# ocrickard/piper-swift

Measured on AMD Instinct MI355X. Metric: audio-sec/wall-sec (RTF^-1) with ms/utterance, Piper VITS en_GB-medium geometry, scale-bench factor, higher is better.
Workload: dtype f32; 1 GPU; medium factor=8: 112 ids, 336 frames, 86016 samples (3.901 s audio) per utterance, 1 utterance per step per GPU; factor=8, phoneme_count=112, frames=336, samples=86016, parallelism=utterance-replicas x1 (one-shot RCCL weight broadcast)

## Files before the change

### piper-swift_amd/csrc/conv_win.h

```cpp
#pragma once
#include "common.h"

namespace ph {

struct ConvWinArgs {
  const float* x = nullptr;
  const float* x2 = nullptr;
  const float* x3 = nullptr;
  const float* w4 = nullptr;
  const float* bias = nullptr;
  const float* res = nullptr;
  const float* mrf_a = nullptr;
  const float* mrf_b = nullptr;
  float* y = nullptr;
  float pro_alpha = 1.0f;
  float out_alpha = 1.0f;
  int N = 1, Cin = 0, Cout = 0, K = 1, dil = 1, padL = 0;
  int Lin = 0;
  int Lout = 0;
  int y_len = 0;
  int ct_stride = 0, ct_pad = 0;
  const int* len_ptr = nullptr;
  int len_mul = 1;
};

size_t packed_conv_win_floats(int Cout, int Cin, int K);
size_t packed_convt_win_floats(int Cin, int Cout, int K, int stride);
int pack_conv_weights_win(hipStream_t s, const float* w, int Cout, int Cin, int K, float* packed);
int pack_convt_weights_win(hipStream_t s, const float* w, int Cin, int Cout, int K, int stride, int pad, float* packed);

bool conv_win_eligible(int Cout, int Cin, int K, int dil, int padL, int Lin, int Lout);
bool convt_win_eligible(int Cin, int Cout, int K, int stride, int pad, int Lin);

int launch_conv_win(piper_hip_ctx* ctx, hipStream_t s, const ConvWinArgs& a);
constexpr int kWinMulti = 3;
int launch_conv_win_multi(piper_hip_ctx* ctx, hipStream_t s, const ConvWinArgs* convs, int count);

size_t packed_conv_pipe_floats(int Cout, int Cin, int K);
size_t packed_convt_pipe_floats(int Cin, int Cout, int K, int stride);
int pack_conv_weights_pipe(hipStream_t s, const float* w, int Cout, int Cin, int K, float* packed);
int pack_convt_weights_pipe(hipStream_t s, const float* w, int Cin, int Cout, int K, int stride, int pad, float* packed);
bool conv_pipe_eligible(int Cout, int Cin, int K, int dil, int padL, int Lin, int Lout);
bool convt_pipe_eligible(int Cin, int Cout, int K, int stride, int pad, int Lin);
int launch_conv_pipe_multi(piper_hip_ctx* ctx, hipStream_t s, const ConvWinArgs* convs, int count);

struct RbPairArgs {
  const float* x = nullptr;
  float* y = nullptr;
  const float *wa4 = nullptr, *ba = nullptr, *wb4 = nullptr, *bb = nullptr;
  int Ka = 1, dila = 1, Kb = 1, dilb = 1;
  int res_a = 1, res_b_x = 0;
  float alpha = 0.1f;
  int N = 1, C = 0, L = 0;
  const int* len_ptr = nullptr;
  int len_mul = 1;
};
bool rb_pair_eligible(int C, int Ka, int dila, int Kb, int dilb, int L);
int launch_rb_pair_multi(piper_hip_ctx* ctx, hipStream_t s, const RbPairArgs* pairs, int count);

}
```

### piper-swift_amd/csrc/conv_win.hip

```cpp
#include <algorithm>
#include <cstdlib>
#include <type_traits>

#include "conv_win.h"

namespace ph {
namespace {

typedef float f32x16 __attribute__((ext_vector_type(16)));

constexpr int kBT = 256;
constexpr int kRA = 8;
constexpr int kStepPad = 16;
constexpr int kTailFloats = 4096;

__device__ __forceinline__ float lrelu1(float v, float alpha) { return v >= 0.0f ? v : v * alpha; }

inline int padded_steps_win(int Cin, int taps) { return (taps * (Cin / 2) + kStepPad - 1) / kStepPad * kStepPad; }

__global__ __launch_bounds__(kBT) void pack_conv_win_kernel(const float* __restrict__ w, int Cout, int Cin, int K, int S, int Sp,
                                                           float* __restrict__ out, int64_t total) {
  const int C2 = Cin >> 1;
  for (int64_t i = (int64_t)blockIdx.x * kBT + threadIdx.x; i < total; i += (int64_t)gridDim.x * kBT) {
    const int e = (int)(i & 3), l = (int)((i >> 2) & 63);
    const int64_t g = i >> 8;
    const int s4 = (int)(g % (Sp >> 2)), mt = (int)(g / (Sp >> 2));
    const int step = 4 * s4 + e;
    float v = 0.0f;
    const int row = mt * 32 + (l & 31);
    if (step < S && row < Cout) {
      const int tap = step / C2, c2 = step - tap * C2;
      v = w[((int64_t)row * Cin + 2 * c2 + (l >> 5)) * K + tap];
    }
    out[i] = v;
  }
}

__global__ __launch_bounds__(kBT) void pack_convt_win_kernel(const float* __restrict__ w, int Cin, int Cout, int K, int stride, int pad,
                                                            int S, int Sp, float* __restrict__ out, int64_t total) {
  const int C2 = Cin >> 1;
  for (int64_t i = (int64_t)blockIdx.x * kBT + threadIdx.x; i < total; i += (int64_t)gridDim.x * kBT) {
    const int e = (int)(i & 3), l = (int)((i >> 2) & 63);
    const int64_t g = i >> 8;
    const int s4 = (int)(g % (Sp >> 2)), mt = (int)(g / (Sp >> 2));
    const int step = 4 * s4 + e;
    float v = 0.0f;
    const int R = mt * 32 + (l & 31);
    const int rho = R / Cout, co = R - rho * Cout;
    if (step < S && rho < stride) {
      const int j = step / C2, c2 = step - j * C2;
      v = w[((int64_t)(2 * c2 + (l >> 5)) * Cout + co) * K + (rho + pad) % stride + stride * j];
    }
    out[i] = v;
  }
}

#ifdef PH_WIN_TRACE
__device__ unsigned long long* ph_win_trace_buf;
#define PH_WSTAMP(k) do { const int bl_ = blockIdx.x + gridDim.x * (blockIdx.y + gridDim.y * blockIdx.z); if ((threadIdx.x & 63) == 0 && ph_win_trace_buf && bl_ < 1024) ph_win_trace_buf[((size_t)bl_ * 4 + (threadIdx.x >> 6)) * 8 + (k)] = __builtin_amdgcn_s_memtime(); } while (0)
#else
#define PH_WSTAMP(k) do { } while (0)
#endif

struct ConvWinMulti {
  ConvWinArgs c[kWinMulti];
};

template <int WM, int WN, int KS>
__global__ __launch_bounds__(64 * WM * WN * KS) void conv_win_kernel(const ConvWinMulti multi, int batch, int xcd_rows) {
  constexpr int NW = WM * WN * KS, BT = 64 * NW;
  extern __shared__ __attribute__((aligned(16))) float win[];
  const ConvWinArgs& p = multi.c[blockIdx.z / batch];
  int bx = blockIdx.x, by = blockIdx.y;
  if (xcd_rows) {
    const int lin = blockIdx.x + gridDim.x * blockIdx.y;
    const int q = lin >> 3;
    const int yh = __builtin_amdgcn_readfirstlane(q / (int)gridDim.x);
    bx = q - yh * (int)gridDim.x;
    by = (lin & 7) + 8 * yh;
  }
  static_assert(NW == 4 || NW == 8, "4 or 8 waves per block");
  constexpr int NBC = WN * 32;
  PH_WSTAMP(0);
  const int lane = threadIdx.x & 63;
  const int wave = __builtin_amdgcn_readfirstlane(threadIdx.x >> 6);
  const int ks = wave / (WM * WN), wt = wave % (WM * WN);
  const int wm = wt % WM, wn = wt / WM;
  const int r = lane & 31, h = lane >> 5;
  const bool ct = p.ct_stride > 0;
  const int taps = ct ? p.K / p.ct_stride : p.K;
  const int C2 = p.Cin >> 1;
  const int n = blockIdx.z % batch;
  const int nb0 = bx * NBC;
  if (p.len_ptr && nb0 >= min(p.len_ptr[n] * p.len_mul, p.Lin)) return;
  const int mt = by * WM + wm;
  const int off_min = ct ? -(taps - 1) : -p.padL;
  const int off_max = ct ? (p.ct_stride - 1 + p.ct_pad) / p.ct_stride : (p.K - 1) * p.dil - p.padL;
  const int W = NBC + off_max - off_min;
  const int g0 = nb0 + off_min;
  const int ga = g0 & ~3;
  const int shift = g0 - ga;
  const int Wp = (W + 3 + 3) & ~3;
  const int S = taps * C2;
  const int Sp = (S + kStepPad - 1) / kStepPad * kStepPad;
  const int Sw = Sp / KS;
  const int s_begin = ks * Sw;

  const char* wa = (const char*)p.w4 + ((int64_t)mt * Sp + s_begin) * 256;
  const unsigned lane16 = (unsigned)lane * 16u;
  float4 a[kRA];
  auto load_a = [&](int slot, int ahead) { a[slot] = *(const float4*)(wa + ahead * 1024 + lane16); };
#pragma unroll
  for (int d = 0; d < kRA - 1; d++) load_a(d, d);

  auto stage = [&](auto avg_tag) {
    constexpr bool AVG = decltype(avg_tag)::value;
    constexpr int kStage = (AVG ? 5 : 16) * 4 / NW + (AVG && NW > 4 ? 1 : 0);
    const int64_t xoff = (int64_t)n * p.Cin * p.Lin;
    const float* xb = p.x + xoff;
    const float* xb2 = AVG ? p.x2 + xoff : nullptr;
    const float* xb3 = AVG ? p.x3 + xoff : nullptr;
    const int W4 = Wp >> 2;
    const int total4 = p.Cin * W4;
    const int dump = p.Cin * Wp;
    const int Lv = p.len_ptr ? min(p.len_ptr[n] * p.len_mul, p.Lin) : p.Lin;
    const unsigned inv = 0xFFFFFFFFu / (unsigned)W4 + 1u;
    for (int base = threadIdx.x; base < total4; base += BT * kStage) {
      float4 t[kStage], t2[AVG ? kStage : 1], t3[AVG ? kStage : 1];
// ... 6 lines not shown
        const int row = (int)__umulhi((unsigned)ic, inv);
        const int i4 = ic - row * W4;
        const int pos = ga + 4 * i4;
        nvalid[q] = pos < 0 ? 0 : Lv - pos;
        const int64_t off = (int64_t)row * p.Lin + ((pos >= 0 && pos < p.Lin) ? pos : 0);
        t[q] = *(const float4*)(xb + off);
        if constexpr (AVG) { t2[q] = *(const float4*)(xb2 + off); t3[q] = *(const float4*)(xb3 + off); }
        dst[q] = i < total4 ? row * Wp + 4 * i4 : dump;
      }
#pragma unroll
      for (int q = 0; q < kStage; q++) {
        float4 v = t[q];
        if constexpr (AVG) {
          v.x = ((v.x + t2[q].x) + t3[q].x) / 3.0f; v.y = ((v.y + t2[q].y) + t3[q].y) / 3.0f;
          v.z = ((v.z + t2[q].z) + t3[q].z) / 3.0f; v.w = ((v.w + t2[q].w) + t3[q].w) / 3.0f;
        }
        v.x = lrelu1(v.x, p.pro_alpha); v.y = lrelu1(v.y, p.pro_alpha); v.z = lrelu1(v.z, p.pro_alpha); v.w = lrelu1(v.w, p.pro_alpha);
        v.x = nvalid[q] > 0 ? v.x : 0.0f; v.y = nvalid[q] > 1 ? v.y : 0.0f; v.z = nvalid[q] > 2 ? v.z : 0.0f; v.w = nvalid[q] > 3 ? v.w : 0.0f;
        *(float4*)(win + dst[q]) = v;
      }
    }
  };
  PH_WSTAMP(1);
  if (p.x2) stage(std::true_type{});
  else stage(std::false_type{});
  PH_WSTAMP(2);
  __syncthreads();
  PH_WSTAMP(3);

  f32x16 acc;
#pragma unroll
  for (int q = 0; q < 16; q++) acc[q] = 0.0f;

  const int rho = ct ? (mt * 32) / p.Cout : 0;
  const int off0 = ct ? (rho + p.ct_pad) / p.ct_stride : -p.padL;
  const int dstep = ct ? -1 : p.dil;
  const int lbase = h * Wp + shift + wn * 32 + r - off_min + off0;
  const int tap0 = s_begin / C2, c20 = s_begin - tap0 * C2;
  int sidx = 2 * c20 * Wp + min(tap0, taps - 1) * dstep;
  int c_n = c20, left = S - 1 - s_begin;
  if (left < 0) sidx = 0;
  const int wrap_delta = dstep - 2 * Wp * (C2 - 1);
  float b[2][4];
  auto read_b4 = [&](int slot) {
#pragma unroll
    for (int e = 0; e < 4; e++) {
      b[slot][e] = win[lbase + sidx];
      c_n++;
      const bool wrap = c_n == C2;
      c_n = wrap ? 0 : c_n;
      const int delta = wrap ? wrap_delta : 2 * Wp;
      sidx += left > 0 ? delta : 0;
      left--;
    }
  };
  auto group = [&](int u) {
    load_a((u + kRA - 1) % kRA, kRA - 1 + u);
    __builtin_amdgcn_sched_barrier(0);
    read_b4((u + 1) & 1);
    acc = __builtin_amdgcn_mfma_f32_32x32x2f32(a[u].x, b[u & 1][0], acc, 0, 0, 0);
    acc = __builtin_amdgcn_mfma_f32_32x32x2f32(a[u].y, b[u & 1][1], acc, 0, 0, 0);
    acc = __builtin_amdgcn_mfma_f32_32x32x2f32(a[u].z, b[u & 1][2], acc, 0, 0, 0);
    acc = __builtin_amdgcn_mfma_f32_32x32x2f32(a[u].w, b[u & 1][3], acc, 0, 0, 0);
  };
  read_b4(0);
  __builtin_amdgcn_s_waitcnt(0x0F70);
  const int G = Sw >> 2;
  const int full = G / kRA;
  for (int g = 0; g < full; g++) {
#pragma unroll
    for (int u = 0; u < kRA; u++) group(u);
    wa += kRA * 1024;
  }
  {
    const int rem = G - full * kRA;
#pragma unroll
    for (int u = 0; u < kRA - 1; u++)
      if (u < rem) group(u);
  }

  PH_WSTAMP(4);
  if constexpr (KS > 1) {
    __syncthreads();
    float* red = win;
    if (ks > 0) {
      float* dst = red + ((ks - 1) * (WM * WN) + wt) * (16 * 64) + lane;
#pragma unroll
      for (int q = 0; q < 16; q++) dst[q * 64] = acc[q];
    }
    __syncthreads();
    if (ks > 0) return;
#pragma unroll
    for (int s2 = 1; s2 < KS; s2++) {
      const float* src = red + ((s2 - 1) * (WM * WN) + wt) * (16 * 64) + lane;
#pragma unroll
      for (int q = 0; q < 16; q++) acc[q] += src[q * 64];
    }
  }

  PH_WSTAMP(5);
  const int rows_total = ct ? p.Cout * p.ct_stride : p.Cout;
  const int row0 = mt * 32;
  if (row0 >= rows_total) return;
  const int co0 = ct ? row0 - rho * p.Cout : row0;
  const int col = nb0 + wn * 32 + r;
  const bool okc = col < p.Lout;
  const int colc = min(col, p.Lout - 1);
  const int pos = ct ? colc * p.ct_stride + rho : colc;
  int64_t yi[16];
  float v[16];
#pragma unroll
  for (int q = 0; q < 16; q++) {
    const int coc = min(co0 + (q & 3) + 8 * (q >> 2) + 4 * h, p.Cout - 1);
    yi[q] = ((int64_t)n * p.Cout + coc) * p.y_len + pos;
    v[q] = acc[q] + (p.bias ? p.bias[coc] : 0.0f);
  }
  if (p.res) {
    float t[16];
#pragma unroll
    for (int q = 0; q < 16; q++) t[q] = p.res[yi[q]];
#pragma unroll
    for (int q = 0; q < 16; q++) v[q] += t[q];
  }
  if (p.mrf_a) {
    float ta[16], tb[16];
#pragma unroll
    for (int q = 0; q < 16; q++) { ta[q] = p.mrf_a[yi[q]]; tb[q] = p.mrf_b[yi[q]]; }
#pragma unroll
    for (int q = 0; q < 16; q++) v[q] = ((ta[q] + tb[q]) + v[q]) / 3.0f;
  }
#pragma unroll
  for (int q = 0; q < 16; q++)
    if (okc && co0 + (q & 3) + 8 * (q >> 2) + 4 * h < p.Cout) p.y[yi[q]] = lrelu1(v[q], p.out_alpha);
  PH_WSTAMP(6);
}

template <int WM, int WN, int KS>
int launch_inst(hipStream_t s, const ConvWinMulti& a, int batch, dim3 grid, size_t lds, int xcd_rows) {
  static bool raised[kMaxDevices] = {};
  if (lds > 64 * 1024 && lds_optin_needed(raised))
    (void)hipFuncSetAttribute((const void*)conv_win_kernel<WM, WN, KS>, hipFuncAttributeMaxDynamicSharedMemorySize, 160 * 1024);
  hipLaunchKernelGGL((conv_win_kernel<WM, WN, KS>), grid, dim3(64 * WM * WN * KS), lds, s, a, batch, xcd_rows);
  return PIPER_HIP_OK;
}

struct WinGeom {
  int MT, taps, reach, per_phase;
};
WinGeom geom(const ConvWinArgs& a) {
  WinGeom g;
  const bool ct = a.ct_stride > 0;
  const int rows = ct ? a.Cout * a.ct_stride : a.Cout;
  g.MT = (rows + 31) / 32;
  g.taps = ct ? a.K / a.ct_stride : a.K;
  g.reach = ct ? (a.ct_stride - 1 + a.ct_pad) / a.ct_stride + g.taps - 1 : (a.K - 1) * a.dil;
  g.per_phase = ct ? a.Cout / 32 : g.MT;
  return g;
}
size_t lds_bytes(int Cin, int wn, int reach, int ks, int wmwn) {
  const int Wp = (wn * 32 + reach + 6) & ~3;
  const size_t window = ((size_t)Cin * Wp + 4) * 4;
  const size_t red = (size_t)(ks - 1) * wmwn * 16 * 64 * 4;
  return window > red ? window : red;
}

}

#ifdef PH_WIN_TRACE
void conv_win_set_trace(unsigned long long* buf) { (void)hipMemcpyToSymbol(HIP_SYMBOL(ph_win_trace_buf), &buf, sizeof buf); }
#endif

size_t packed_conv_win_floats(int Cout, int Cin, int K) { return (size_t)((Cout + 31) / 32) * padded_steps_win(Cin, K) * 64 + kTailFloats; }
size_t packed_convt_win_floats(int Cin, int Cout, int K, int stride) {
  return (size_t)((Cout * stride + 31) / 32) * padded_steps_win(Cin, K / stride) * 64 + kTailFloats;
}

int pack_conv_weights_win(hipStream_t s, const float* w, int Cout, int Cin, int K, float* packed) {
  const int64_t total = (int64_t)packed_conv_win_floats(Cout, Cin, K);
  const int grid = (int)std::min<int64_t>(ceil_div(total, kBT), 4096);
  hipLaunchKernelGGL(pack_conv_win_kernel, dim3(grid), dim3(kBT), 0, s, w, Cout, Cin, K, K * (Cin / 2), padded_steps_win(Cin, K), packed, total);
  return PIPER_HIP_OK;
}
int pack_convt_weights_win(hipStream_t s, const float* w, int Cin, int Cout, int K, int stride, int pad, float* packed) {
  const int64_t total = (int64_t)packed_convt_win_floats(Cin, Cout, K, stride);
  const int grid = (int)std::min<int64_t>(ceil_div(total, kBT), 4096);
  const int J = K / stride;
  hipLaunchKernelGGL(pack_convt_win_kernel, dim3(grid), dim3(kBT), 0, s, w, Cin, Cout, K, stride, pad, J * (Cin / 2), padded_steps_win(Cin, J),
                     packed, total);
  return PIPER_HIP_OK;
}

bool conv_win_eligible(int Cout, int Cin, int K, int dil, int padL, int Lin, int Lout) {
  if (Cout < 1 || Cin < 2 || (Cin & 1) || K < 1 || dil < 1 || padL < 0 || Lin < 4 || (Lin & 3) || Lout < 1) return false;
  return lds_bytes(Cin, 1, (K - 1) * dil, 1, 1) <= 160 * 1024;
}
bool convt_win_eligible(int Cin, int Cout, int K, int stride, int pad, int Lin) {
  if (Cin < 2 || (Cin & 1) || Cout < 32 || (Cout & 31) || stride < 1 || Lin < 4 || (Lin & 3)) return false;
  return K % stride == 0 && K - stride == 2 * pad;
}

int launch_conv_win(piper_hip_ctx* ctx, hipStream_t s, const ConvWinArgs& a) { return launch_conv_win_multi(ctx, s, &a, 1); }

int launch_conv_win_multi(piper_hip_ctx* ctx, hipStream_t s, const ConvWinArgs* convs, int count) {
  if (count < 1 || count > kWinMulti) PH_FAIL(PIPER_HIP_ERR_ARG, "conv_win: %d convs in one launch (1..%d)", count, kWinMulti);
  const ConvWinArgs& a = convs[0];
  if (a.N <= 0 || a.Lout <= 0) return PIPER_HIP_OK;
  const WinGeom g = geom(a);
  int reach = g.reach, Sp_min = padded_steps_win(a.Cin, g.taps);
  for (int i = 1; i < count; i++) {
    const ConvWinArgs& b = convs[i];
    if (b.N != a.N || b.Cin != a.Cin || b.Cout != a.Cout || b.Lin != a.Lin || b.Lout != a.Lout || b.ct_stride != a.ct_stride)
      PH_FAIL(PIPER_HIP_ERR_SHAPE, "conv_win: convs of one launch must share N, Cin, Cout, Lin, Lout and kind");
    const WinGeom gb = geom(b);
    reach = std::max(reach, gb.reach);
    Sp_min = std::min(Sp_min, padded_steps_win(b.Cin, gb.taps));
  }
  const int64_t tiles = (int64_t)g.MT * ceil_div(a.Lout, 32) * a.N * count;
  const int64_t simds = 4 * (int64_t)ctx->num_cus;
  static const bool ks_one_wave = getenv("PIPER_HIP_WIN_KS_ONE_WAVE") != nullptr;
  int KS = ks_one_wave ? (tiles >= simds ? 1 : (2 * tiles >= simds ? 2 : 4)) : (tiles >= 2 * simds ? 1 : (tiles >= simds ? 2 : 4));
  while (KS > 1 && Sp_min / KS < 16) KS >>= 1;
  static const int cand[7][3] = {{4, 1, 1}, {2, 2, 1}, {1, 4, 1}, {2, 1, 2}, {1, 2, 2}, {1, 1, 4}, {4, 1, 2}};
  constexpr int kCand4 = 6;
  int best = -1;
  static const char* force = getenv("PIPER_HIP_WIN_CFG");
  int fm = 0, fn = 0, fk = 0;
  const bool forced = force && sscanf(force, "%d,%d,%d", &fm, &fn, &fk) == 3;
  if (!forced && a.ct_stride == 0 && g.MT % 4 == 0 && a.Cin >= 128 && KS == 4 && Sp_min / 2 >= 16 && lds_bytes(a.Cin, 1, reach, 2, 4) <= 160 * 1024) best = 6;
  for (int pass = 0; pass < 3 && best < 0; pass++)
    for (int i = 0; i < (pass == 0 ? 7 : kCand4) && best < 0; i++) {
      const int m = cand[i][0], nn = cand[i][1], k = cand[i][2];
      if (g.MT % m || (k > 1 && Sp_min / k < 16) || lds_bytes(a.Cin, nn, reach, k, m * nn) > 160 * 1024) continue;
      if (pass == 0 && !(forced && m == fm && nn == fn && k == fk)) continue;
      if (pass == 1 && k != KS) continue;
      best = i;
    }
  if (best < 0) PH_FAIL(PIPER_HIP_ERR_UNSUPPORTED, "conv_win: no configuration fits (Cin=%d reach=%d rows/phase=%d)", a.Cin, reach, g.per_phase);
  const int WM = cand[best][0], WN = cand[best][1];
  KS = cand[best][2];
  const size_t lds = lds_bytes(a.Cin, WN, reach, KS, WM * WN);
  const dim3 grid((unsigned)ceil_div(a.Lout, WN * 32), (unsigned)ceil_div(g.MT, WM), (unsigned)(a.N * count));
  ConvWinMulti multi;
  for (int i = 0; i < kWinMulti; i++) multi.c[i] = convs[i < count ? i : 0];
  static const bool no_xcd = getenv("PIPER_HIP_WIN_NO_XCD_ROWS") != nullptr;
  const int64_t w_bytes = (int64_t)g.MT * Sp_min * 256, x_bytes = (int64_t)a.Cin * a.Lin * 4 * (a.x2 ? 3 : 1);
  const int xcd_rows = (!no_xcd && grid.y % 8 == 0 && w_bytes > x_bytes) ? 1 : 0;
#define PH_WIN_CASE(M, N_, K_) \
  if (WM == M && WN == N_ && KS == K_) launch_inst<M, N_, K_>(s, multi, a.N, grid, lds, xcd_rows); else
  PH_WIN_CASE(4, 1, 1) PH_WIN_CASE(2, 2, 1) PH_WIN_CASE(1, 4, 1) PH_WIN_CASE(2, 1, 2) PH_WIN_CASE(1, 2, 2) PH_WIN_CASE(1, 1, 4)
  PH_WIN_CASE(4, 1, 2)
  PH_FAIL(PIPER_HIP_ERR_UNSUPPORTED, "conv_win: no instance for WM=%d WN=%d KS=%d", WM, WN, KS);
#undef PH_WIN_CASE
  for (int i = 0; i < count; i++)
    PH_ROUTE(ctx, convs[i].Cout, convs[i].Cin, convs[i].Lout, convs[i].N, "win K=%d WM=%d WN=%d KS=%d multi=%d xcd=%d avg3=%d %s", convs[i].K, WM, WN, KS, count,
             xcd_rows, convs[i].x2 ? 1 : 0, a.ct_stride > 0 ? "convT" : "conv");
  hipError_t e = hipGetLastError();
  if (e != hipSuccess) PH_FAIL(PIPER_HIP_ERR_LAUNCH, "conv_win launch failed: %s", hipGetErrorString(e));
  return PIPER_HIP_OK;
}

}
namespace ph { namespace { PH_WARM(conv_win, pack_conv_win_kernel); } }
```

### piper-swift_amd/csrc/ops_conv.cpp

```cpp
#include "conv.h"
#include "conv_bf16.h"
#include "conv_win.h"

using namespace ph;

namespace {
int pool_floats(piper_hip_ctx* ctx, size_t n, float** out) {
  void* p = nullptr;
  int rc = ctx->pool.alloc(n * sizeof(float), &p);
  if (rc) return rc;
  *out = (float*)p;
  return PIPER_HIP_OK;
}
bool fits_i32(int64_t v) { return v >= 0 && v <= 0x7fffffff; }
}

PH_EXPORT int piper_hip_conv1d_f32(piper_hip_ctx* ctx, const float* x, const int64_t x_shape[3], const float* w,
                                   const int64_t w_shape[3], const float* bias, const piper_hip_conv1d_params* p,
                                   float** out, int64_t out_shape[3], piper_hip_stream stream) {
  PH_CHECK_CTX(ctx);
  if (!x_shape || !w_shape || !p) PH_FAIL(PIPER_HIP_ERR_ARG, "conv1dF32: null shape/params");
  const int64_t N = x_shape[0], Cin = x_shape[1], Lin = x_shape[2];
  const int64_t Cout = w_shape[0], K = w_shape[2];
  const int64_t g = p->groups < 1 ? 1 : p->groups;
// ... 65 lines not shown
  const int64_t N = x_shape[0], Cin = x_shape[1], Lin = x_shape[2];
  const int64_t g = p->groups < 1 ? 1 : p->groups;
  if (N < 0 || Cin < 0 || Lin < 0 || w_shape[1] < 0 || w_shape[2] <= 0) PH_FAIL(PIPER_HIP_ERR_SHAPE, "convTranspose1dF32: bad dimension");
  if (p->stride < 1 || p->dilation < 1 || p->pad_l < 0 || p->pad_r < 0 || p->output_padding < 0)
    PH_FAIL(PIPER_HIP_ERR_SHAPE, "convTranspose1dF32: stride/dilation must be >=1 and pads >=0");
  if (Cin % g) PH_FAIL(PIPER_HIP_ERR_SHAPE, "convTranspose1dF32 invalid groups: C_in=%lld groups=%lld", (long long)Cin, (long long)g);
  if (w_shape[0] != Cin) PH_FAIL(PIPER_HIP_ERR_SHAPE, "convTranspose1dF32 weight[0] mismatch: %lld vs C_in=%lld", (long long)w_shape[0], (long long)Cin);
  const int64_t cog = w_shape[1], Cout = cog * g, K = w_shape[2];
  const int64_t Lout = (Lin - 1) * p->stride - p->pad_l - p->pad_r + (int64_t)p->dilation * (K - 1) + p->output_padding + 1;
  if (Lout <= 0) PH_FAIL(PIPER_HIP_ERR_SHAPE, "convTranspose1dF32 produced invalid L_out=%lld", (long long)Lout);
  if (out_shape) { out_shape[0] = N; out_shape[1] = Cout; out_shape[2] = Lout; }
  const int64_t count = N * Cout * Lout;
  if (!fits_i32(Cin * Lin) || !fits_i32(Cout * Lout) || !fits_i32(Cin * cog * K))
    PH_FAIL(PIPER_HIP_ERR_SHAPE, "convTranspose1dF32: tensor too large for 32-bit indexing");
  int rc = ensure_out(ctx, out, (size_t)count, 0);
  if (rc) return rc;
  if (count == 0) return PIPER_HIP_OK;
  if (!x || !w) PH_FAIL(PIPER_HIP_ERR_ARG, "convTranspose1dF32: null input");
  StreamScope ss(ctx, stream);
  RouteScope routes(ctx);
  const int s = p->stride;
  static const bool no_win = getenv("PIPER_HIP_NO_WIN") != nullptr;
  if (!no_win && g == 1 && p->dilation == 1 && p->output_padding == 0 && p->pad_l == p->pad_r && Lin >= 256 &&
      ((uintptr_t)x & 15) == 0 && convt_win_eligible((int)Cin, (int)Cout, (int)K, s, p->pad_l, (int)Lin)) {
    static const bool no_pipe = getenv("PIPER_HIP_NO_PIPE") != nullptr;
    static const double pipe_ct_min = [] { const char* e = getenv("PIPER_HIP_PIPE_CT_MIN_GFLOP"); return e ? atof(e) * 1e9 : 1e30; }();
    const bool pipe = !no_pipe && 2.0 * (double)Cout * (double)Cin * (double)K * (double)Lin * (double)N >= pipe_ct_min &&
                      convt_pipe_eligible((int)Cin, (int)Cout, (int)K, s, p->pad_l, (int)Lin);
    float* packed = nullptr;
    rc = pool_floats(ctx, pipe ? packed_convt_pipe_floats((int)Cin, (int)Cout, (int)K, s) : packed_convt_win_floats((int)Cin, (int)Cout, (int)K, s), &packed);
    if (rc) return rc;
    defer_free(ctx, packed);
    if (pipe) pack_convt_weights_pipe(ss.s, w, (int)Cin, (int)Cout, (int)K, s, p->pad_l, packed);
    else pack_convt_weights_win(ss.s, w, (int)Cin, (int)Cout, (int)K, s, p->pad_l, packed);
    ConvWinArgs wa;
    wa.x = x; wa.w4 = packed; wa.bias = bias; wa.y = *out;
    wa.N = (int)N; wa.Cin = (int)Cin; wa.Cout = (int)Cout; wa.K = (int)K; wa.Lin = (int)Lin; wa.Lout = (int)Lin; wa.y_len = (int)Lout;
    wa.ct_stride = s; wa.ct_pad = p->pad_l;
    rc = pipe ? launch_conv_pipe_multi(ctx, ss.s, &wa, 1) : launch_conv_win(ctx, ss.s, wa);
  } else if (g == 1 && p->dilation == 1 && Cin >= 2 && Cout * s >= 8 && Lin >= 1) {
    const int J = (int)((K + s - 1) / s);
    const int Lg = (int)((Lout - 1 + p->pad_l) / s + 1);
    const int tm = conv_pick_tile(ctx, (int)(Cout * s), Lg, (int)N, 0);
    float* packed = nullptr;
    rc = pool_floats(ctx, packed_convt_floats((int)Cin, (int)Cout, (int)K, s, tm), &packed);
    if (rc) return rc;
    defer_free(ctx, packed);
    pack_convt_weights(ss.s, w, (int)Cin, (int)Cout, (int)K, s, packed, tm);
    ConvArgs a;
    a.x = x; a.bias = bias; a.y = *out;
    if (tm == 16) a.w16 = packed; else a.w = packed;
    a.N = (int)N; a.Cin = (int)Cin; a.Cout = (int)(Cout * s); a.K = J; a.dil = -1; a.padL = 0;
    a.Lin = (int)Lin; a.Lout = (int)((Lout - 1 + p->pad_l) / s + 1);
    a.x_batch_stride = Cin * Lin; a.y_batch_stride = Cout * Lout; a.y_len = (int)Lout;
    a.epilogue = EPI_CONVT; a.ct_stride = s; a.ct_padL = p->pad_l; a.ct_Lout = (int)Lout;
    rc = launch_conv_mfma(ctx, ss.s, a);
  } else {
    rc = launch_convt_direct(ctx, ss.s, x, w, bias, *out, (int)N, (int)Cin, (int)Lin, (int)Cout, (int)K, s, p->dilation,
                             p->pad_l, (int)Lout, (int)g);
  }
  if (rc) return rc;
  return ss.finish("convtranspose1d_f32");
}

PH_EXPORT int piper_hip_conv1d_bf16(piper_hip_ctx* ctx, const float* x, const int64_t x_shape[3], const float* w,
                                    const int64_t w_shape[3], const float* bias, const piper_hip_conv1d_params* p,
                                    float** out, int64_t out_shape[3], piper_hip_stream stream) {
  PH_CHECK_CTX(ctx);
  if (!x_shape || !w_shape || !p) PH_FAIL(PIPER_HIP_ERR_ARG, "conv1dBF16: null shape/params");
  const int64_t N = x_shape[0], Cin = x_shape[1], Lin = x_shape[2];
  const int64_t Cout = w_shape[0], K = w_shape[2];
// ... 237 lines not shown
```

### piper-swift_amd/csrc/voice.hip

```cpp
#include <algorithm>
#include <cmath>
#include <cstdlib>
#include <chrono>
#include <functional>
#include <memory>

#include "../../include/piper_hip_voice_layout.h"
#include "conv.h"
#include "conv_bf16.h"
#include "conv_win.h"
#include "pcm16.h"
#include "resample.h"
#include "rng.h"
#include "speaker.h"

namespace ph {
int validate_config(const piper_hip_voice_config* c);
int validate_speaker_config(const piper_hip_voice_config* cfg, const piper_hip_speaker_config* sc);
int launch_rel_attention(piper_hip_ctx* ctx, hipStream_t s, const float* q, const float* k, const float* v, const float* ek,
                         const float* ev, float* out, int N, int H, int d, int T, int w, int64_t in_batch_stride,
                         int64_t out_batch_stride, const int* len_ptr);
int rel_attention_split_parts(piper_hip_ctx* ctx, int N, int H, int d, int T, int w);
int launch_rel_attention_split(piper_hip_ctx* ctx, hipStream_t s, const float* q, const float* k, const float* v, const float* ek,
                               const float* ev, float* out, int N, int H, int d, int T, int w, int64_t in_batch_stride,
// ... 127 lines not shown
      (void)hipGetLastError();
      if (clk::now() - t0 > std::chrono::milliseconds(5)) break;
      for (int i = 0; i < 16; i++) __builtin_ia32_pause();
    }
  }
  return hipStreamSynchronize(q);
}

struct Step {
  std::string name;
  std::function<int(hipStream_t)> run;
  double flops = 0, bytes = 0;
  std::string tag;
  int lane = 0;
  enum Kind { LAUNCH, FORK, JOIN } kind = LAUNCH;
  piper_hip_ctx* ctx = nullptr;
  std::string routes;
  int enqueue(hipStream_t q) {
    if (__builtin_expect(!ctx->routes_on, 1)) return run(q);
    routes.clear();
    ctx->route_sink = &routes;
    const int rc = run(q);
    ctx->route_sink = nullptr;
    return rc;
  }
};

struct ConvW {
  const float* w = nullptr;
  const float* w16 = nullptr;
  const float* w16g = nullptr;
  const float* w8 = nullptr;
  const float* w4 = nullptr;
  const float* w5 = nullptr;
  const float* bias = nullptr;
  int Cout = 0, Cin = 0, K = 1;
  bool mfma = false;
};

struct StreamSet {
  hipStream_t stream = nullptr, side[2] = {nullptr, nullptr};
  hipEvent_t ev0 = nullptr, ev1 = nullptr, ev_fork = nullptr, ev_join[2] = {nullptr, nullptr};
};

enum PlanKind : int {
  PLAN_WHOLE = 0,
  PLAN_GENERATOR = 1,
  PLAN_PREDICT = 2,
  PLAN_FROM_STATS = 3,
};

struct RowFormat {
  int rate = 0, enc = PIPER_HIP_ENC_S16;
  float gain = 1.0f;
};

struct StreamRow {
  int F = 0, next = 0;
  bool active = false;
  bool ghost = false;
  RowFormat fmt;
};

struct StreamRate {
  int rate = 0;
  bool started = false;
// ... 337 lines not shown
    double* scratch = (double*)pk.take(2 * flow_tail_scratch_doubles(H, half));
    for (int f = 0; f < c.n_flows; f++) {
      auto& C = v->flows[f];
      const int seam = f > 0;
      float* img = pk.take(flow_tail_image_floats(H, half, seam));
      float* tb = pk.take((size_t)half + (seam ? H : 0));
      if (dry) continue;
      auto raw = [&](const char* what, int g) {
        snprintf(nm, sizeof nm, "flow.flows.%d.%s", 2 * g, what);
        return std::string(nm);
      };
      const std::string rs = raw("enc.res_skip_layers.", f) + std::to_string(c.wn_layers - 1), post = raw("post", f), pre = raw("pre", std::max(f - 1, 0));
      const int rc = fold_flow_tail(pk.s, tensor(v, rs + ".weight"), tensor(v, rs + ".bias"), tensor(v, post + ".weight"), tensor(v, post + ".bias"),
                                    seam ? tensor(v, pre + ".weight") : nullptr, seam ? tensor(v, pre + ".bias") : nullptr, H, half,
                                    (c.n_flows - f) % 2 ? -1 : 1, scratch, img, tb);
      if (rc) return rc;
      C.tail_w = img; C.tail_b = tb;
    }
  }
  v->conv_pre = make_conv(pk, dry, "dec.conv_pre", c.up_initial, I, 7);
  int ch = c.up_initial;
  for (int u = 0; u < c.n_ups; u++) {
    piper_hip_voice::Stage S;
    S.Cin = ch; S.Cout = ch / 2; S.K = c.up_kernels[u]; S.stride = c.up_rates[u]; S.pad = (S.K - S.stride) / 2;
    const int J = (S.K + S.stride - 1) / S.stride;
    S.up.Cout = S.Cout * S.stride; S.up.Cin = S.Cin; S.up.K = J; S.up.mfma = true;
    float* p = pk.take(packed_convt_floats(S.Cin, S.Cout, S.K, S.stride));
    float* p16 = pk.take(packed_convt_floats(S.Cin, S.Cout, S.K, S.stride, 16));
    S.up.w = p;
    S.up.w16 = p16;
    const bool ct_win = convt_win_eligible(S.Cin, S.Cout, S.K, S.stride, S.pad, 4);
    float* p4 = ct_win ? pk.take(packed_convt_win_floats(S.Cin, S.Cout, S.K, S.stride)) : nullptr;
    S.up.w4 = ct_win ? p4 : nullptr;
    const bool ct_pipe = convt_pipe_eligible(S.Cin, S.Cout, S.K, S.stride, S.pad, 4);
    float* p5 = ct_pipe ? pk.take(packed_convt_pipe_floats(S.Cin, S.Cout, S.K, S.stride)) : nullptr;
    S.up.w5 = p5;
    if (!dry) {
      snprintf(nm, sizeof nm, "dec.ups.%d", u);
      if (ct_win) pack_convt_weights_win(pk.s, tensor(v, std::string(nm) + ".weight"), S.Cin, S.Cout, S.K, S.stride, S.pad, p4);
      if (ct_pipe) pack_convt_weights_pipe(pk.s, tensor(v, std::string(nm) + ".weight"), S.Cin, S.Cout, S.K, S.stride, S.pad, p5);
      pack_convt_weights(pk.s, tensor(v, std::string(nm) + ".weight"), S.Cin, S.Cout, S.K, S.stride, p);
      pack_convt_weights(pk.s, tensor(v, std::string(nm) + ".weight"), S.Cin, S.Cout, S.K, S.stride, p16, 16);
      S.up.bias = tensor(v, std::string(nm) + ".bias");
    }
    ch /= 2;
    for (int j = 0; j < c.n_rb; j++) {
      std::vector<ConvW> convs;
      const int rb = u * c.n_rb + j;
      for (int d = 0; d < c.rb_n_dil; d++) {
        if (c.resblock_type == 1) {
          snprintf(nm, sizeof nm, "dec.resblocks.%d.convs1.%d", rb, d);
          convs.push_back(make_conv(pk, dry, nm, ch, ch, c.rb_kernels[j], true, true));
          snprintf(nm, sizeof nm, "dec.resblocks.%d.convs2.%d", rb, d);
          convs.push_back(make_conv(pk, dry, nm, ch, ch, c.rb_kernels[j], true, true));
        } else {
          snprintf(nm, sizeof nm, "dec.resblocks.%d.convs.%d", rb, d);
          convs.push_back(make_conv(pk, dry, nm, ch, ch, c.rb_kernels[j], true, true));
        }
      }
      S.rb.push_back(convs);
    }
    v->stages.push_back(S);
  }
  v->conv_post = make_conv(pk, dry, "dec.conv_post", 1, ch, 7, false);
  v->dp.clear();
  if (c.dp_present) {
    auto dds_of = [&](const std::string& base) {
      std::vector<piper_hip_voice::DdsLayer> out;
      for (int i = 0; i < c.dp_dds_layers; i++) {
        piper_hip_voice::DdsLayer d{};
        const std::string sep = base + ".convs.convs_sep." + std::to_string(i), n1 = base + ".convs.norms_1." + std::to_string(i),
                          n2 = base + ".convs.norms_2." + std::to_string(i);
// ... 259 lines not shown
  }
};
const GenF32Switches& gen_f32_switches() {
  static const GenF32Switches sw;
  return sw;
}


ConvWinArgs win_args(const Builder& b, const ConvW& w, const float* x, const float* res, float* y, int dil, int L, const float* mrf_a = nullptr,
                     const float* mrf_b = nullptr, float out_alpha = 1.0f) {
  ConvWinArgs wa;
  wa.x = x; wa.w4 = w.w4; wa.bias = w.bias; wa.res = res; wa.y = y;
  wa.pro_alpha = 0.1f;
  if (mrf_a) { wa.mrf_a = mrf_a; wa.mrf_b = mrf_b; wa.out_alpha = out_alpha; }
  wa.N = b.NB; wa.Cin = w.Cin; wa.Cout = w.Cout; wa.K = w.K; wa.dil = dil; wa.padL = (w.K * dil - dil) / 2;
  wa.Lin = L; wa.Lout = L; wa.y_len = L;
  wa.len_ptr = b.lensF; wa.len_mul = L / b.F;
  return wa;
}

void add_convt_f32(Builder& b, const std::string& name, const piper_hip_voice::Stage& S, const float* const cur[3], float pro_alpha, float* up,
                   int L) {
  const GenF32Switches& sw = gen_f32_switches();
  piper_hip_ctx* ctx = b.v->ctx;
  const int NB = b.NB, Lo = L * S.stride;
  const double flops = NB * 2.0 * S.Cin * S.Cout * (double)S.K * L;
  const double bytes = NB * 4.0 * ((double)S.Cin * L * (cur[1] ? 3 : 1) + (double)S.Cout * Lo + (double)S.Cin * S.Cout * S.K + S.Cout);
  const bool pipe = sw.use_win && sw.pipe_pays(flops, S.Cin, true) && S.up.w5 && convt_pipe_eligible(S.Cin, S.Cout, S.K, S.stride, S.pad, L);
  if (pipe || (sw.use_win && S.up.w4 && convt_win_eligible(S.Cin, S.Cout, S.K, S.stride, S.pad, L))) {
    ConvWinArgs wa;
    wa.x = cur[0]; wa.x2 = cur[1]; wa.x3 = cur[2]; wa.w4 = pipe ? S.up.w5 : S.up.w4; wa.bias = S.up.bias; wa.y = up;
    wa.pro_alpha = pro_alpha;
    wa.N = NB; wa.Cin = S.Cin; wa.Cout = S.Cout; wa.K = S.K; wa.Lin = L; wa.Lout = L; wa.y_len = Lo;
    wa.ct_stride = S.stride; wa.ct_pad = S.pad;
    wa.len_ptr = b.lensF; wa.len_mul = L / b.F;
    if (pipe) b.step(name, "conv_mfma", flops, bytes, [ctx, wa](hipStream_t q) { return launch_conv_pipe_multi(ctx, q, &wa, 1); });
    else b.step(name, "conv_mfma", flops, bytes, [ctx, wa](hipStream_t q) { return launch_conv_win(ctx, q, wa); });
    return;
  }
  ConvArgs a;
  a.x = cur[0]; a.x2 = cur[1]; a.x3 = cur[2];
  a.prologue = cur[1] ? PRO_AVG3_LRELU : pro_alpha == 1.0f ? PRO_NONE : PRO_LRELU;
  a.alpha = 0.1f;
  a.y = up; a.N = NB; a.dil = -1; a.padL = 0; a.Lin = L; a.Lout = (Lo - 1 + S.pad) / S.stride + 1;
  a.len_ptr = b.lensF; a.len_mul = L / b.F;
  a.x_batch_stride = (int64_t)S.Cin * L; a.y_batch_stride = (int64_t)S.Cout * Lo; a.y_len = Lo;
  a.epilogue = EPI_CONVT; a.ct_stride = S.stride; a.ct_padL = S.pad; a.ct_Lout = Lo;
  a.w = S.up.w; a.w16 = S.up.w16; a.bias = S.up.bias; a.Cin = S.up.Cin; a.Cout = S.up.Cout; a.K = S.up.K;
  b.step(name, "conv_mfma", flops, bytes, [ctx, a](hipStream_t q) { return launch_conv_mfma(ctx, q, a); });
}

void add_mrf_mean(Builder& b, const std::string& name, const float* r0, const float* r1, const float* r2, float* y, int64_t cnt, float alpha) {
  b.step(name, "", 0, 0, [=](hipStream_t q) {
    const int grid = (int)std::min<int64_t>(ceil_div(cnt, (int64_t)kBlock * 4), 2048);
    hipLaunchKernelGGL(mrf_mean_lrelu_kernel, dim3(grid), dim3(kBlock), 0, q, r0, r1, r2, y, cnt, alpha);
    return PIPER_HIP_OK;
  });
}

int add_conv_post(Builder& b, const std::string& name, const float* x, const float* x2, const float* x3, int prologue, int L) {
  Slot& s = b.s;
  s.n_samples = L;
  s.audio = b.ar.f32((size_t)b.NB * L);
  if (b.ar.rc) return b.ar.rc;
  b.tap("audio", s.audio, 1, L, L / b.F);
  ConvArgs a;
  a.x = x; a.x2 = x2; a.x3 = x3;
// ... 3804 lines not shown
```

Baseline: 5789 audio-sec/wall-sec.

## Interleave transposed-conv phases per row tile and split K-slice epilogue across waves

Repacks transposed-conv weights so each 32-row MFMA tile holds several stride phases of fewer output channels (4 phases for stride 8, 2 for stride 4). This lets the epilogue write contiguous float4/float2 runs of the upsampled output instead of strided scalar stores. It also adds a shared-memory epilogue for split-K configs: every K-slice wave stores its partials and then reduces and stores a 1/KS share of the outputs, instead of wave 0 doing all of it. The cost is a larger reduction buffer in LDS, remapped tile indices under the XCD row swizzle, and more complex index math.

```diff
diff --git a/piper-swift_amd/csrc/conv_win.h b/piper-swift_amd/csrc/conv_win.h
--- a/piper-swift_amd/csrc/conv_win.h
+++ b/piper-swift_amd/csrc/conv_win.h
@@ -20,6 +20,7 @@
   int Lout = 0;
   int y_len = 0;
   int ct_stride = 0, ct_pad = 0;
+  int ct_rows = 1;
   const int* len_ptr = nullptr;
   int len_mul = 1;
 };
@@ -27,7 +28,8 @@
 size_t packed_conv_win_floats(int Cout, int Cin, int K);
 size_t packed_convt_win_floats(int Cin, int Cout, int K, int stride);
 int pack_conv_weights_win(hipStream_t s, const float* w, int Cout, int Cin, int K, float* packed);
-int pack_convt_weights_win(hipStream_t s, const float* w, int Cin, int Cout, int K, int stride, int pad, float* packed);
+int convt_win_rows(int Cout, int K, int stride, int pad, int y_len);
+int pack_convt_weights_win(hipStream_t s, const float* w, int Cin, int Cout, int K, int stride, int pad, float* packed, int rows = 1);
 
 bool conv_win_eligible(int Cout, int Cin, int K, int dil, int padL, int Lin, int Lout);
 bool convt_win_eligible(int Cin, int Cout, int K, int stride, int pad, int Lin);
diff --git a/piper-swift_amd/csrc/conv_win.hip b/piper-swift_amd/csrc/conv_win.hip
--- a/piper-swift_amd/csrc/conv_win.hip
+++ b/piper-swift_amd/csrc/conv_win.hip
@@ -37,7 +37,7 @@
 }
 
 __global__ __launch_bounds__(kBT) void pack_convt_win_kernel(const float* __restrict__ w, int Cin, int Cout, int K, int stride, int pad,
-                                                            int S, int Sp, float* __restrict__ out, int64_t total) {
+                                                            int S, int Sp, int rows, float* __restrict__ out, int64_t total) {
   const int C2 = Cin >> 1;
   for (int64_t i = (int64_t)blockIdx.x * kBT + threadIdx.x; i < total; i += (int64_t)gridDim.x * kBT) {
     const int e = (int)(i & 3), l = (int)((i >> 2) & 63);
@@ -46,7 +46,13 @@
     const int step = 4 * s4 + e;
     float v = 0.0f;
     const int R = mt * 32 + (l & 31);
-    const int rho = R / Cout, co = R - rho * Cout;
+    int rho = R / Cout, co = R - rho * Cout;
+    if (rows > 1) {
+      const int ti = l & 31;
+      rho = rows * (mt & 1) + (ti & (rows - 1));
+      co = (32 / rows) * (mt >> 1) + ti / rows;
+      if (co >= Cout) rho = stride;
+    }
     if (step < S && rho < stride) {
       const int j = step / C2, c2 = step - j * C2;
       v = w[((int64_t)(2 * c2 + (l >> 5)) * Cout + co) * K + (rho + pad) % stride + stride * j];
@@ -66,8 +72,13 @@
   ConvWinArgs c[kWinMulti];
 };
 
+constexpr int kWinXcdRows = 1;
+constexpr int kWinEpiShared = 2;
+constexpr int kWinCtVec = 4;
+
 template <int WM, int WN, int KS>
-__global__ __launch_bounds__(64 * WM * WN * KS) void conv_win_kernel(const ConvWinMulti multi, int batch, int xcd_rows) {
+__global__ __launch_bounds__(64 * WM * WN * KS) void conv_win_kernel(const ConvWinMulti multi, int batch, int flags) {
+  const int xcd_rows = flags & kWinXcdRows;
   constexpr int NW = WM * WN * KS, BT = 64 * NW;
   extern __shared__ __attribute__((aligned(16))) float win[];
   const ConvWinArgs& p = multi.c[blockIdx.z / batch];
@@ -93,7 +104,10 @@
   const int n = blockIdx.z % batch;
   const int nb0 = bx * NBC;
   if (p.len_ptr && nb0 >= min(p.len_ptr[n] * p.len_mul, p.Lin)) return;
-  const int mt = by * WM + wm;
+  const int G = ct ? p.ct_rows : 1;
+  const int lg = G == 4 ? 2 : G == 2 ? 1 : 0;
+  int mt = by * WM + wm;
+  if (G > 1 && WM == 1 && xcd_rows && (gridDim.y & 15) == 0) mt = 2 * ((mt & 7) + 8 * (mt >> 4)) + ((mt >> 3) & 1);
   const int off_min = ct ? -(taps - 1) : -p.padL;
   const int off_max = ct ? (p.ct_stride - 1 + p.ct_pad) / p.ct_stride : (p.K - 1) * p.dil - p.padL;
   const int W = NBC + off_max - off_min;
@@ -166,7 +180,7 @@
 #pragma unroll
   for (int q = 0; q < 16; q++) acc[q] = 0.0f;
 
-  const int rho = ct ? (mt * 32) / p.Cout : 0;
+  const int rho = !ct ? 0 : G > 1 ? G * (mt & 1) : (mt * 32) / p.Cout;
   const int off0 = ct ? (rho + p.ct_pad) / p.ct_stride : -p.padL;
   const int dstep = ct ? -1 : p.dil;
   const int lbase = h * Wp + shift + wn * 32 + r - off_min + off0;
@@ -199,24 +213,99 @@
   };
   read_b4(0);
   __builtin_amdgcn_s_waitcnt(0x0F70);
-  const int G = Sw >> 2;
-  const int full = G / kRA;
+  const int groups = Sw >> 2;
+  const int full = groups / kRA;
   for (int g = 0; g < full; g++) {
 #pragma unroll
     for (int u = 0; u < kRA; u++) group(u);
     wa += kRA * 1024;
   }
   {
-    const int rem = G - full * kRA;
+    const int rem = groups - full * kRA;
 #pragma unroll
     for (int u = 0; u < kRA - 1; u++)
       if (u < rem) group(u);
   }
 
   PH_WSTAMP(4);
+  const int rows_total = ct ? p.Cout * p.ct_stride : p.Cout;
+  const int row0 = mt * 32;
+  const int co0 = !ct ? row0 : G > 1 ? (mt >> 1) * (32 >> lg) : row0 - rho * p.Cout;
+  const int vecw = (flags & kWinCtVec) ? G : 1;
+  auto finish = [&](auto nq_tag, const float* sum, int q0) {
+    constexpr int NQ = decltype(nq_tag)::value;
+    if (row0 >= rows_total) return;
+    const int col = nb0 + wn * 32 + r;
+    const bool okc = col < p.Lout;
+    const int colc = min(col, p.Lout - 1);
+    const int pos = ct ? colc * p.ct_stride + rho : colc;
+    int64_t yi[NQ];
+    float v[NQ];
+#pragma unroll
+    for (int qq = 0; qq < NQ; qq++) {
+      const int q = q0 + qq, i = (q & 3) + 8 * (q >> 2) + 4 * h;
+      const int coc = min(co0 + (i >> lg), p.Cout - 1);
+      yi[qq] = ((int64_t)n * p.Cout + coc) * p.y_len + pos + (i & (G - 1));
+      v[qq] = sum[qq] + (p.bias ? p.bias[coc] : 0.0f);
+    }
+    if (p.res) {
+      float t[NQ];
+#pragma unroll
+      for (int qq = 0; qq < NQ; qq++) t[qq] = p.res[yi[qq]];
+#pragma unroll
+      for (int qq = 0; qq < NQ; qq++) v[qq] += t[qq];
+    }
+    if (p.mrf_a) {
+      float ta[NQ], tb[NQ];
+#pragma unroll
+      for (int qq = 0; qq < NQ; qq++) { ta[qq] = p.mrf_a[yi[qq]]; tb[qq] = p.mrf_b[yi[qq]]; }
+#pragma unroll
+      for (int qq = 0; qq < NQ; qq++) v[qq] = ((ta[qq] + tb[qq]) + v[qq]) / 3.0f;
+    }
+#pragma unroll
+    for (int qq = 0; qq < NQ; qq++) v[qq] = lrelu1(v[qq], p.out_alpha);
+    auto ok = [&](int qq) {
+      const int q = q0 + qq;
+      return okc && co0 + (((q & 3) + 8 * (q >> 2) + 4 * h) >> lg) < p.Cout;
+    };
+    if (vecw == 4) {
+#pragma unroll
+      for (int qq = 0; qq < NQ; qq += 4)
+        if (ok(qq)) *(float4*)(p.y + yi[qq]) = make_float4(v[qq], v[qq + 1], v[qq + 2], v[qq + 3]);
+    } else if (vecw == 2) {
+#pragma unroll
+      for (int qq = 0; qq < NQ; qq += 2)
+        if (ok(qq)) *(float2*)(p.y + yi[qq]) = make_float2(v[qq], v[qq + 1]);
+    } else {
+#pragma unroll
+      for (int qq = 0; qq < NQ; qq++)
+        if (ok(qq)) p.y[yi[qq]] = v[qq];
+    }
+  };
+
   if constexpr (KS > 1) {
     __syncthreads();
     float* red = win;
+    if (flags & kWinEpiShared) {
+      constexpr int NQ = 16 / KS;
+      float* dst = red + (ks * (WM * WN) + wt) * (16 * 64) + lane;
+#pragma unroll
+      for (int q = 0; q < 16; q++) dst[q * 64] = acc[q];
+      __syncthreads();
+      const int q0 = ks * NQ;
+      const float* src = red + (wt * 16 + q0) * 64 + lane;
+      float part[NQ];
+#pragma unroll
+      for (int qq = 0; qq < NQ; qq++) part[qq] = src[qq * 64];
+#pragma unroll
+      for (int s2 = 1; s2 < KS; s2++)
+#pragma unroll
+        for (int qq = 0; qq < NQ; qq++) part[qq] += src[s2 * (WM * WN) * (16 * 64) + qq * 64];
+      PH_WSTAMP(5);
+      finish(std::integral_constant<int, NQ>{}, part, q0);
+      PH_WSTAMP(6);
+      return;
+    }
     if (ks > 0) {
       float* dst = red + ((ks - 1) * (WM * WN) + wt) * (16 * 64) + lane;
 #pragma unroll
@@ -233,48 +322,19 @@
   }
 
   PH_WSTAMP(5);
-  const int rows_total = ct ? p.Cout * p.ct_stride : p.Cout;
-  const int row0 = mt * 32;
-  if (row0 >= rows_total) return;
-  const int co0 = ct ? row0 - rho * p.Cout : row0;
-  const int col = nb0 + wn * 32 + r;
-  const bool okc = col < p.Lout;
-  const int colc = min(col, p.Lout - 1);
-  const int pos = ct ? colc * p.ct_stride + rho : colc;
-  int64_t yi[16];
-  float v[16];
-#pragma unroll
-  for (int q = 0; q < 16; q++) {
-    const int coc = min(co0 + (q & 3) + 8 * (q >> 2) + 4 * h, p.Cout - 1);
-    yi[q] = ((int64_t)n * p.Cout + coc) * p.y_len + pos;
-    v[q] = acc[q] + (p.bias ? p.bias[coc] : 0.0f);
-  }
-  if (p.res) {
-    float t[16];
-#pragma unroll
-    for (int q = 0; q < 16; q++) t[q] = p.res[yi[q]];
-#pragma unroll
-    for (int q = 0; q < 16; q++) v[q] += t[q];
-  }
-  if (p.mrf_a) {
-    float ta[16], tb[16];
-#pragma unroll
-    for (int q = 0; q < 16; q++) { ta[q] = p.mrf_a[yi[q]]; tb[q] = p.mrf_b[yi[q]]; }
-#pragma unroll
-    for (int q = 0; q < 16; q++) v[q] = ((ta[q] + tb[q]) + v[q]) / 3.0f;
-  }
-#pragma unroll
-  for (int q = 0; q < 16; q++)
-    if (okc && co0 + (q & 3) + 8 * (q >> 2) + 4 * h < p.Cout) p.y[yi[q]] = lrelu1(v[q], p.out_alpha);
+  float a16[16];
+#pragma unroll
+  for (int q = 0; q < 16; q++) a16[q] = acc[q];
+  finish(std::integral_constant<int, 16>{}, a16, 0);
   PH_WSTAMP(6);
 }
 
 template <int WM, int WN, int KS>
-int launch_inst(hipStream_t s, const ConvWinMulti& a, int batch, dim3 grid, size_t lds, int xcd_rows) {
+int launch_inst(hipStream_t s, const ConvWinMulti& a, int batch, dim3 grid, size_t lds, int flags) {
   static bool raised[kMaxDevices] = {};
   if (lds > 64 * 1024 && lds_optin_needed(raised))
     (void)hipFuncSetAttribute((const void*)conv_win_kernel<WM, WN, KS>, hipFuncAttributeMaxDynamicSharedMemorySize, 160 * 1024);
-  hipLaunchKernelGGL((conv_win_kernel<WM, WN, KS>), grid, dim3(64 * WM * WN * KS), lds, s, a, batch, xcd_rows);
+  hipLaunchKernelGGL((conv_win_kernel<WM, WN, KS>), grid, dim3(64 * WM * WN * KS), lds, s, a, batch, flags);
   return PIPER_HIP_OK;
 }
 
@@ -291,10 +351,10 @@
   g.per_phase = ct ? a.Cout / 32 : g.MT;
   return g;
 }
-size_t lds_bytes(int Cin, int wn, int reach, int ks, int wmwn) {
+size_t lds_bytes(int Cin, int wn, int reach, int ks, int wmwn, bool shared = false) {
   const int Wp = (wn * 32 + reach + 6) & ~3;
   const size_t window = ((size_t)Cin * Wp + 4) * 4;
-  const size_t red = (size_t)(ks - 1) * wmwn * 16 * 64 * 4;
+  const size_t red = (size_t)(ks > 1 && shared ? ks : ks - 1) * wmwn * 16 * 64 * 4;
   return window > red ? window : red;
 }
 
@@ -315,12 +375,18 @@
   hipLaunchKernelGGL(pack_conv_win_kernel, dim3(grid), dim3(kBT), 0, s, w, Cout, Cin, K, K * (Cin / 2), padded_steps_win(Cin, K), packed, total);
   return PIPER_HIP_OK;
 }
-int pack_convt_weights_win(hipStream_t s, const float* w, int Cin, int Cout, int K, int stride, int pad, float* packed) {
+int convt_win_rows(int Cout, int K, int stride, int pad, int y_len) {
+  static const bool plain = getenv("PIPER_HIP_CT_ROWS_PLAIN") != nullptr;
+  if (plain || stride < 1 || K != 2 * stride || 2 * pad != stride || (Cout & 31) || (y_len & 3)) return 1;
+  return stride == 8 ? 4 : stride == 4 ? 2 : 1;
+}
+int pack_convt_weights_win(hipStream_t s, const float* w, int Cin, int Cout, int K, int stride, int pad, float* packed, int rows) {
+  if (rows != 1 && rows != convt_win_rows(Cout, K, stride, pad, 4)) PH_FAIL(PIPER_HIP_ERR_ARG, "conv_win: %d phases per row tile do not fit K=%d stride=%d pad=%d Cout=%d", rows, K, stride, pad, Cout);
   const int64_t total = (int64_t)packed_convt_win_floats(Cin, Cout, K, stride);
   const int grid = (int)std::min<int64_t>(ceil_div(total, kBT), 4096);
   const int J = K / stride;
   hipLaunchKernelGGL(pack_convt_win_kernel, dim3(grid), dim3(kBT), 0, s, w, Cin, Cout, K, stride, pad, J * (Cin / 2), padded_steps_win(Cin, J),
-                     packed, total);
+                     rows, packed, total);
   return PIPER_HIP_OK;
 }
 
@@ -343,7 +409,8 @@
   int reach = g.reach, Sp_min = padded_steps_win(a.Cin, g.taps);
   for (int i = 1; i < count; i++) {
     const ConvWinArgs& b = convs[i];
-    if (b.N != a.N || b.Cin != a.Cin || b.Cout != a.Cout || b.Lin != a.Lin || b.Lout != a.Lout || b.ct_stride != a.ct_stride)
+    if (b.N != a.N || b.Cin != a.Cin || b.Cout != a.Cout || b.Lin != a.Lin || b.Lout != a.Lout || b.ct_stride != a.ct_stride ||
+        b.ct_rows != a.ct_rows)
       PH_FAIL(PIPER_HIP_ERR_SHAPE, "conv_win: convs of one launch must share N, Cin, Cout, Lin, Lout and kind");
     const WinGeom gb = geom(b);
     reach = std::max(reach, gb.reach);
@@ -358,13 +425,15 @@
   constexpr int kCand4 = 6;
   int best = -1;
   static const char* force = getenv("PIPER_HIP_WIN_CFG");
+  static const bool epi_slice0 = getenv("PIPER_HIP_WIN_EPI_SLICE0") != nullptr;
+  const bool shared = !epi_slice0;
   int fm = 0, fn = 0, fk = 0;
   const bool forced = force && sscanf(force, "%d,%d,%d", &fm, &fn, &fk) == 3;
-  if (!forced && a.ct_stride == 0 && g.MT % 4 == 0 && a.Cin >= 128 && KS == 4 && Sp_min / 2 >= 16 && lds_bytes(a.Cin, 1, reach, 2, 4) <= 160 * 1024) best = 6;
+  if (!forced && a.ct_stride == 0 && g.MT % 4 == 0 && a.Cin >= 128 && KS == 4 && Sp_min / 2 >= 16 && lds_bytes(a.Cin, 1, reach, 2, 4, shared) <= 160 * 1024) best = 6;
   for (int pass = 0; pass < 3 && best < 0; pass++)
     for (int i = 0; i < (pass == 0 ? 7 : kCand4) && best < 0; i++) {
       const int m = cand[i][0], nn = cand[i][1], k = cand[i][2];
-      if (g.MT % m || (k > 1 && Sp_min / k < 16) || lds_bytes(a.Cin, nn, reach, k, m * nn) > 160 * 1024) continue;
+      if (g.MT % m || (k > 1 && Sp_min / k < 16) || lds_bytes(a.Cin, nn, reach, k, m * nn, shared) > 160 * 1024) continue;
       if (pass == 0 && !(forced && m == fm && nn == fn && k == fk)) continue;
       if (pass == 1 && k != KS) continue;
       best = i;
@@ -372,15 +441,23 @@
   if (best < 0) PH_FAIL(PIPER_HIP_ERR_UNSUPPORTED, "conv_win: no configuration fits (Cin=%d reach=%d rows/phase=%d)", a.Cin, reach, g.per_phase);
   const int WM = cand[best][0], WN = cand[best][1];
   KS = cand[best][2];
-  const size_t lds = lds_bytes(a.Cin, WN, reach, KS, WM * WN);
+  const size_t lds = lds_bytes(a.Cin, WN, reach, KS, WM * WN, shared);
   const dim3 grid((unsigned)ceil_div(a.Lout, WN * 32), (unsigned)ceil_div(g.MT, WM), (unsigned)(a.N * count));
   ConvWinMulti multi;
   for (int i = 0; i < kWinMulti; i++) multi.c[i] = convs[i < count ? i : 0];
   static const bool no_xcd = getenv("PIPER_HIP_WIN_NO_XCD_ROWS") != nullptr;
   const int64_t w_bytes = (int64_t)g.MT * Sp_min * 256, x_bytes = (int64_t)a.Cin * a.Lin * 4 * (a.x2 ? 3 : 1);
   const int xcd_rows = (!no_xcd && grid.y % 8 == 0 && w_bytes > x_bytes) ? 1 : 0;
+  int flags = (xcd_rows ? kWinXcdRows : 0) | (shared ? kWinEpiShared : 0);
+  if (a.ct_stride > 0 && a.ct_rows != 1) {
+    if (a.ct_rows != convt_win_rows(a.Cout, a.K, a.ct_stride, a.ct_pad, 4))
+      PH_FAIL(PIPER_HIP_ERR_ARG, "conv_win: ct_rows=%d does not fit K=%d stride=%d pad=%d Cout=%d", a.ct_rows, a.K, a.ct_stride, a.ct_pad, a.Cout);
+    bool vec = true;
+    for (int i = 0; i < count; i++) vec = vec && (convs[i].y_len & 3) == 0 && ((uintptr_t)convs[i].y & 15) == 0;
+    if (vec) flags |= kWinCtVec;
+  }
 #define PH_WIN_CASE(M, N_, K_) \
-  if (WM == M && WN == N_ && KS == K_) launch_inst<M, N_, K_>(s, multi, a.N, grid, lds, xcd_rows); else
+  if (WM == M && WN == N_ && KS == K_) launch_inst<M, N_, K_>(s, multi, a.N, grid, lds, flags); else
   PH_WIN_CASE(4, 1, 1) PH_WIN_CASE(2, 2, 1) PH_WIN_CASE(1, 4, 1) PH_WIN_CASE(2, 1, 2) PH_WIN_CASE(1, 2, 2) PH_WIN_CASE(1, 1, 4)
   PH_WIN_CASE(4, 1, 2)
   PH_FAIL(PIPER_HIP_ERR_UNSUPPORTED, "conv_win: no instance for WM=%d WN=%d KS=%d", WM, WN, KS);
diff --git a/piper-swift_amd/csrc/ops_conv.cpp b/piper-swift_amd/csrc/ops_conv.cpp
--- a/piper-swift_amd/csrc/ops_conv.cpp
+++ b/piper-swift_amd/csrc/ops_conv.cpp
@@ -121,11 +121,12 @@
     if (rc) return rc;
     defer_free(ctx, packed);
     if (pipe) pack_convt_weights_pipe(ss.s, w, (int)Cin, (int)Cout, (int)K, s, p->pad_l, packed);
-    else pack_convt_weights_win(ss.s, w, (int)Cin, (int)Cout, (int)K, s, p->pad_l, packed);
+    const int rows = pipe ? 1 : convt_win_rows((int)Cout, (int)K, s, p->pad_l, (int)Lout);
+    if (!pipe) pack_convt_weights_win(ss.s, w, (int)Cin, (int)Cout, (int)K, s, p->pad_l, packed, rows);
     ConvWinArgs wa;
     wa.x = x; wa.w4 = packed; wa.bias = bias; wa.y = *out;
     wa.N = (int)N; wa.Cin = (int)Cin; wa.Cout = (int)Cout; wa.K = (int)K; wa.Lin = (int)Lin; wa.Lout = (int)Lin; wa.y_len = (int)Lout;
-    wa.ct_stride = s; wa.ct_pad = p->pad_l;
+    wa.ct_stride = s; wa.ct_pad = p->pad_l; wa.ct_rows = rows;
     rc = pipe ? launch_conv_pipe_multi(ctx, ss.s, &wa, 1) : launch_conv_win(ctx, ss.s, wa);
   } else if (g == 1 && p->dilation == 1 && Cin >= 2 && Cout * s >= 8 && Lin >= 1) {
     const int J = (int)((K + s - 1) / s);
diff --git a/piper-swift_amd/csrc/voice.hip b/piper-swift_amd/csrc/voice.hip
--- a/piper-swift_amd/csrc/voice.hip
+++ b/piper-swift_amd/csrc/voice.hip
@@ -183,6 +183,7 @@
   const float* w16g = nullptr;
   const float* w8 = nullptr;
   const float* w4 = nullptr;
+  int ct_rows = 1;
   const float* w5 = nullptr;
   const float* bias = nullptr;
   int Cout = 0, Cin = 0, K = 1;
@@ -586,12 +587,13 @@
     const bool ct_win = convt_win_eligible(S.Cin, S.Cout, S.K, S.stride, S.pad, 4);
     float* p4 = ct_win ? pk.take(packed_convt_win_floats(S.Cin, S.Cout, S.K, S.stride)) : nullptr;
     S.up.w4 = ct_win ? p4 : nullptr;
+    S.up.ct_rows = ct_win ? convt_win_rows(S.Cout, S.K, S.stride, S.pad, 4) : 1;
     const bool ct_pipe = convt_pipe_eligible(S.Cin, S.Cout, S.K, S.stride, S.pad, 4);
     float* p5 = ct_pipe ? pk.take(packed_convt_pipe_floats(S.Cin, S.Cout, S.K, S.stride)) : nullptr;
     S.up.w5 = p5;
     if (!dry) {
       snprintf(nm, sizeof nm, "dec.ups.%d", u);
-      if (ct_win) pack_convt_weights_win(pk.s, tensor(v, std::string(nm) + ".weight"), S.Cin, S.Cout, S.K, S.stride, S.pad, p4);
+      if (ct_win) pack_convt_weights_win(pk.s, tensor(v, std::string(nm) + ".weight"), S.Cin, S.Cout, S.K, S.stride, S.pad, p4, S.up.ct_rows);
       if (ct_pipe) pack_convt_weights_pipe(pk.s, tensor(v, std::string(nm) + ".weight"), S.Cin, S.Cout, S.K, S.stride, S.pad, p5);
       pack_convt_weights(pk.s, tensor(v, std::string(nm) + ".weight"), S.Cin, S.Cout, S.K, S.stride, p);
       pack_convt_weights(pk.s, tensor(v, std::string(nm) + ".weight"), S.Cin, S.Cout, S.K, S.stride, p16, 16);
@@ -917,7 +919,7 @@
     wa.x = cur[0]; wa.x2 = cur[1]; wa.x3 = cur[2]; wa.w4 = pipe ? S.up.w5 : S.up.w4; wa.bias = S.up.bias; wa.y = up;
     wa.pro_alpha = pro_alpha;
     wa.N = NB; wa.Cin = S.Cin; wa.Cout = S.Cout; wa.K = S.K; wa.Lin = L; wa.Lout = L; wa.y_len = Lo;
-    wa.ct_stride = S.stride; wa.ct_pad = S.pad;
+    wa.ct_stride = S.stride; wa.ct_pad = S.pad; wa.ct_rows = pipe ? 1 : S.up.ct_rows;
     wa.len_ptr = b.lensF; wa.len_mul = L / b.F;
     if (pipe) b.step(name, "conv_mfma", flops, bytes, [ctx, wa](hipStream_t q) { return launch_conv_pipe_multi(ctx, q, &wa, 1); });
     else b.step(name, "conv_mfma", flops, bytes, [ctx, wa](hipStream_t q) { return launch_conv_win(ctx, q, wa); });
```

New measurement: 5814 audio-sec/wall-sec, median of 6. About the same (+0.4%).
